# Algy/fast-slic

Measured on NVIDIA H100. Metric: megapixels/sec (10 iters, K=1600), higher is better.
Workload: dtype u8/u16 integer

## Files before the change

### fast_slic_b200/csrc/cca.cuh

```cuda
#pragma once
#include "common.cuh"

#define CCA_BLOCK 1024
#define CCA_HIST 2052

struct CcaParams {
    int H, W, N;
    int K;
    int thres;
    int nblk;
    int heap_in_smem;
    int sel_sync;
    int which;
};

__device__ __forceinline__ bool cca_skip_image(const CcaParams& cp, const struct CcaCounters* ct);

struct CcaCounters {
    int ncomp;
    int ncand;
    int nkept;
    int sel_mode;
    int keep_thres;
    int need_sim;
    int dbg_ops;
    int dbg_t;
};

__device__ __forceinline__ bool cca_skip_image(const CcaParams& cp, const CcaCounters* ct) {
    return cp.which >= 0 && (ct->need_sim != 0) != (cp.which != 0);
}

__device__ __forceinline__ int ccl_find(const int* par, int x) {
    int p = par[x];
    while (p != x) {
        x = p;
        p = par[x];
    }
    return x;
}

__device__ __forceinline__ void ccl_union(int* par, int a, int b) {
    a = ccl_find(par, a);
    b = ccl_find(par, b);
    while (a != b) {
        if (a < b) {
            int t = a;
            a = b;
            b = t;
        }
        const int old = atomicMin(&par[a], b);
        if (old == a) break;
        a = ccl_find(par, old);
        b = ccl_find(par, b);
    }
}

#define CCL_T 32
__device__ __forceinline__ int ccl_find_s(const int* par, int x) {
    int p = par[x];
    while (p != x) {
        x = p;
        p = par[x];
    }
    return x;
}
__device__ __forceinline__ void ccl_union_s(int* par, int a, int b) {
    a = ccl_find_s(par, a);
    b = ccl_find_s(par, b);
    while (a != b) {
        if (a < b) {
            int t = a;
            a = b;
            b = t;
        }
        const int old = atomicMin(&par[a], b);
        if (old == a) break;
        a = ccl_find_s(par, old);
        b = ccl_find_s(par, b);
    }
}

#define CCL_TW 4
__global__ void __launch_bounds__(32 * CCL_TW) k_ccl_tile(CcaParams cp, const uint16_t* __restrict__ labels,
                                                          int* __restrict__ par_all, uint32_t* __restrict__ area_all,
                                                          int tiles_x, int tiles_y, long ntiles_total) {
    __shared__ int s_par_all[CCL_TW][CCL_T * CCL_T];
    const int lane = threadIdx.x & 31, warp = threadIdx.x >> 5;
    const long tile = (long)blockIdx.x * CCL_TW + warp;
    if (tile >= ntiles_total) return;
    int* s_par = s_par_all[warp];
    const int per_img = tiles_x * tiles_y;
    const int b = (int)(tile / per_img);
    const int tl = (int)(tile - (long)b * per_img);
    const int tyb = tl / tiles_x, txb = tl - tyb * tiles_x;
    const int j = txb * CCL_T + lane;
    const bool colok = j < cp.W;
    const int nrows = min(CCL_T, cp.H - tyb * CCL_T);
    const uint16_t* lab = labels + (size_t)b * cp.N + (size_t)(tyb * CCL_T) * cp.W + j;
    constexpr int CCL_G = 8;
    uint32_t v[CCL_G], nv[CCL_G];
#pragma unroll
    for (int k = 0; k < CCL_G; k++) {
        v[k] = (colok && k < nrows) ? (uint32_t)lab[(size_t)k * cp.W] : (0x10000u + (uint32_t)(k * CCL_T + lane));
    }
    uint32_t up_v = 0xffffffffu, up_left = 0xffffffffu;
    int up_root = 0;
#pragma unroll 1
    for (int ty0 = 0; ty0 < CCL_T; ty0 += CCL_G) {
#pragma unroll
        for (int k = 0; k < CCL_G; k++) {
            const int ty = ty0 + CCL_G + k;
            nv[k] = (colok && ty < nrows) ? (uint32_t)lab[(size_t)ty * cp.W] : (0x10000u + (uint32_t)((ty & (CCL_T - 1)) * CCL_T + lane));
        }
#pragma unroll
        for (int k = 0; k < CCL_G; k++) {
            const int ty = ty0 + k;
            const uint32_t cur = v[k];
            const uint32_t left = __shfl_up_sync(FSLIC_FULL, cur, 1);
            const bool start = (lane == 0) || (cur != left);
            const unsigned m = __ballot_sync(FSLIC_FULL, start);
            const int sl = 31 - __clz(m & (0xffffffffu >> (31 - lane)));
            const unsigned above = (lane == 31) ? 0u : (m >> (lane + 1));
            const int end = above ? (lane + __ffs(above) - 1) : 31;
            const bool conn = (ty > 0) && (up_v == cur);
            const bool need = conn && ((lane == 0) || (left != cur) || (up_left != up_v));
            unsigned cand = 0xffffffffu;
            if (need) cand = (unsigned)ccl_find_s(s_par, up_root);
            unsigned pm = cand;
#pragma unroll
            for (int o = 1; o < 32; o <<= 1) {
                const unsigned y = __shfl_up_sync(FSLIC_FULL, pm, o);
                if (lane - o >= sl) pm = min(pm, y);
            }
            const unsigned rmin = __shfl_sync(FSLIC_FULL, pm, end);
            const unsigned own = (unsigned)(ty * CCL_T + sl);
            const int root = (int)(rmin < own ? rmin : own);
            if (need && cand != (unsigned)root) ccl_union_s(s_par, (int)cand, root);
            s_par[ty * CCL_T + lane] = root;
            __syncwarp();
            up_left = left;
            up_v = cur;
            up_root = root;
        }
#pragma unroll
        for (int k = 0; k < CCL_G; k++) v[k] = nv[k];
    }
    if (!colok) return;
    int* pout = par_all + (size_t)b * cp.N + (size_t)(tyb * CCL_T) * cp.W + j;
    uint32_t* aout = area_all + (size_t)b * cp.N + (size_t)(tyb * CCL_T) * cp.W + j;
#pragma unroll 4
    for (int ty = 0; ty < nrows; ty++) {
        const int rt = ccl_find_s(s_par, ty * CCL_T + lane);
        const int ri = tyb * CCL_T + (rt >> 5), rj = txb * CCL_T + (rt & 31);
        pout[(size_t)ty * cp.W] = ri * cp.W + rj;
        aout[(size_t)ty * cp.W] = 0;
    }
}

__global__ void __launch_bounds__(256) k_ccl_seams(CcaParams cp, const uint16_t* __restrict__ labels,
                                                   int* __restrict__ par_all) {
    const int b = blockIdx.y;
    const int W = cp.W, H = cp.H;
    const int sv = (W - 1) / CCL_T, sh = (H - 1) / CCL_T;
    const int nV = sv * H, nH = sh * W;
    const uint16_t* lab = labels + (size_t)b * cp.N;
    int* par = par_all + (size_t)b * cp.N;
    for (int t = blockIdx.x * blockDim.x + threadIdx.x; t < nV + nH; t += gridDim.x * blockDim.x) {
        if (t < nV) {
            const int i = t / sv, j = (t - i * sv + 1) * CCL_T;
            const int p = i * W + j;
            if (lab[p - 1] == lab[p]) ccl_union(par, p - 1, p);
        } else {
            const int u = t - nV;
            const int r = u / W, j = u - r * W;
            const int i = (r + 1) * CCL_T;
            const int p = i * W + j;
            const uint16_t v = lab[p], up = lab[p - W];
            if (up == v) {
                bool need = (j % CCL_T == 0) || (lab[p - 1] != v);
                if (!need) need = lab[p - W - 1] != up;
                if (need) ccl_union(par, p - W, p);
            }
        }
    }
}

__global__ void __launch_bounds__(256) k_ccl_flatten(CcaParams cp, const uint16_t* __restrict__ labels,
                                                     int* __restrict__ par_all, uint32_t* __restrict__ area_all,
                                                     int* __restrict__ blkcnt, int* __restrict__ rootbuf_all) {
    __shared__ int s_chunk[32];
    const int b = blockIdx.y;
    const int lane = threadIdx.x & 31, w = threadIdx.x >> 5;
    const uint16_t* lab = labels + (size_t)b * cp.N;
    int* par = par_all + (size_t)b * cp.N;
    int p[4], sl[4], root[4];
    unsigned m[4], rmask[4];
    bool ok[4], start[4], col0[4];
    int jcol = (blockIdx.x * CCA_BLOCK + w * 128 + lane) % cp.W;
#pragma unroll
    for (int r = 0; r < 4; r++) {
        p[r] = blockIdx.x * CCA_BLOCK + (w * 4 + r) * 32 + lane;
        ok[r] = p[r] < cp.N;
        const uint32_t v = ok[r] ? lab[p[r]] : 0x10000u;
        const uint32_t left = __shfl_up_sync(FSLIC_FULL, v, 1);
        const int j = jcol;
        col0[r] = j == 0;
        jcol += 32;
        if (jcol >= cp.W) jcol = (cp.W >= 32) ? (jcol - cp.W) : (jcol % cp.W);
        start[r] = (lane == 0) || (j == 0) || (v != left);
        m[r] = __ballot_sync(FSLIC_FULL, start[r]);
        sl[r] = 31 - __clz(m[r] & (0xffffffffu >> (31 - lane)));
    }
    {
        int q[4];
#pragma unroll
        for (int r = 0; r < 4; r++) {
            root[r] = p[r];
            q[r] = (ok[r] && start[r]) ? par[p[r]] : p[r];
        }
        for (;;) {
            bool mv[4], any = false;
#pragma unroll
            for (int r = 0; r < 4; r++) {
                mv[r] = q[r] != root[r];
                root[r] = q[r];
                any |= mv[r];
            }
            if (!any) break;
#pragma unroll
            for (int r = 0; r < 4; r++)
                if (mv[r]) q[r] = par[root[r]];
        }
    }
#pragma unroll
    for (int r = 0; r < 4; r++) {
        const int rt = __shfl_sync(FSLIC_FULL, root[r], sl[r]);
        bool isroot = false;
        if (ok[r]) {
            par[p[r]] = rt;
            if (start[r]) {
                const unsigned above = (lane == 31) ? 0u : (m[r] >> (lane + 1));
                int len = above ? (__ffs(above)) : (32 - lane);
                if (p[r] + len > cp.N) len = cp.N - p[r];
                atomicAdd(&area_all[(size_t)b * cp.N + rt], (uint32_t)len);
                isroot = (rt == p[r]);
            }
        }
        rmask[r] = __ballot_sync(FSLIC_FULL, isroot);
        if (lane == 0) s_chunk[w * 4 + r] = __popc(rmask[r]);
    }
    __syncthreads();
    const int mine = s_chunk[lane];
    int incl = mine;
#pragma unroll
    for (int o = 1; o < 32; o <<= 1) {
        const int y = __shfl_up_sync(FSLIC_FULL, incl, o);
        if (lane >= o) incl += y;
    }
    int* rootbuf = rootbuf_all + (size_t)b * cp.N + (size_t)blockIdx.x * CCA_BLOCK;
#pragma unroll
    for (int r = 0; r < 4; r++) {
        const int base = __shfl_sync(FSLIC_FULL, incl - mine, w * 4 + r);
        if ((rmask[r] >> lane) & 1u)
            rootbuf[base + __popc(rmask[r] & ((1u << lane) - 1u))] = p[r] | (col0[r] ? (int)0x80000000 : 0);
    }
    if (threadIdx.x == 31) blkcnt[(size_t)b * cp.nblk + blockIdx.x] = incl;
}

__global__ void __launch_bounds__(1024) k_scan_blocks(const int* __restrict__ cnt_all, int* __restrict__ off_all,
                                                      int stride_per_image, int n_static,
                                                      const int* __restrict__ n_dev_base, int n_dev_stride_ints,
                                                      int n_div, int* __restrict__ total_base,
                                                      int total_stride_ints,
                                                      const CcaCounters* __restrict__ skip_counters, int which) {
    __shared__ int s_warp[32];
    __shared__ int s_carry;
    const int b = blockIdx.x;
    if (skip_counters && which >= 0 && (skip_counters[b].need_sim != 0) != (which != 0)) return;
    const int tid = threadIdx.x;
    const int* cnt = cnt_all + (size_t)b * stride_per_image;
    int* off = off_all + (size_t)b * stride_per_image;
    int n = n_static;
    if (n_dev_base) n = (n_dev_base[(size_t)b * n_dev_stride_ints] + n_div - 1) / n_div;
    if (tid == 0) s_carry = 0;
    __syncthreads();
    for (int base = 0; base < n; base += 1024) {
        const int c = base + tid;
        const int v = (c < n) ? cnt[c] : 0;
        int x = v;
#pragma unroll
        for (int o = 1; o < 32; o <<= 1) {
            int y = __shfl_up_sync(FSLIC_FULL, x, o);
            if ((tid & 31) >= o) x += y;
        }
        if ((tid & 31) == 31) s_warp[tid >> 5] = x;
        __syncthreads();
        if (tid < 32) {
            int w = s_warp[tid];
#pragma unroll
            for (int o = 1; o < 32; o <<= 1) {
                int y = __shfl_up_sync(FSLIC_FULL, w, o);
                if (tid >= o) w += y;
            }
            s_warp[tid] = w;
        }
        __syncthreads();
        const int woff = (tid >> 5) ? s_warp[(tid >> 5) - 1] : 0;
        const int excl = s_carry + woff + x - v;
        if (c < n) off[c] = excl;
        __syncthreads();
        if (tid == 1023) s_carry = excl + v;
        __syncthreads();
    }
    if (tid == 0) total_base[(size_t)b * total_stride_ints] = s_carry;
}

#define CCA_NUMBER_GRID 16
__global__ void __launch_bounds__(CCA_BLOCK) k_ccl_number(CcaParams cp, const int* __restrict__ rootbuf_all,
                                                          uint32_t* __restrict__ aux_all,
                                                          const int* __restrict__ blkcnt,
                                                          const int* __restrict__ blkoff,
                                                          int* __restrict__ cleader_all,
                                                          uint32_t* __restrict__ carea_all,
                                                          CcaCounters* __restrict__ counters,
                                                          unsigned int* __restrict__ ahist_all) {
    __shared__ int s_cand;
    __shared__ unsigned int s_hot[CCA_BLOCK / 32][32];
    const int b = blockIdx.y;
    const int lane = threadIdx.x & 31, warp = threadIdx.x >> 5;
    s_hot[warp][lane] = 0;
    if (threadIdx.x == 0) s_cand = 0;
    __syncthreads();
    uint32_t* aux = aux_all + (size_t)b * cp.N;
    int ncand = 0;
    constexpr int NU = 8;
    const int wpi = gridDim.x * (CCA_BLOCK / 32);
    const int NB = (cp.nblk + wpi - 1) / wpi;
    for (int blk0 = (blockIdx.x * (CCA_BLOCK / 32) + warp) * NB; blk0 < cp.nblk; blk0 += wpi * NB) {
        for (int sub = 0; sub < NB; sub += 32) {
            const int myblk = blk0 + sub + lane;
            const bool have = (sub + lane < NB) && (myblk < cp.nblk);
            const int mycnt = have ? blkcnt[(size_t)b * cp.nblk + myblk] : 0;
            const int myoff = have ? blkoff[(size_t)b * cp.nblk + myblk] : 0;
            int incl = mycnt;
#pragma unroll
            for (int o = 1; o < 32; o <<= 1) {
                const int y = __shfl_up_sync(FSLIC_FULL, incl, o);
                if (lane >= o) incl += y;
            }
            const int total = __shfl_sync(FSLIC_FULL, incl, 31);
            const int nb_here = min(32, NB - sub);
            for (int r0 = 0; r0 < total; r0 += 32 * NU) {
                int pp[NU], cc[NU];
                uint32_t aa[NU];
#pragma unroll
                for (int u = 0; u < NU; u++) {
                    const int r = r0 + 32 * u + lane;
                    int bi = 0;
                    for (int q = 0; q < nb_here - 1; q++) bi += (r >= __shfl_sync(FSLIC_FULL, incl, q));
                    const int bincl = __shfl_sync(FSLIC_FULL, incl, bi), bcnt = __shfl_sync(FSLIC_FULL, mycnt, bi);
                    const int boff = __shfl_sync(FSLIC_FULL, myoff, bi);
                    const int t = r - (bincl - bcnt);
                    pp[u] = -1;
                    if (r < total) {
                        pp[u] = rootbuf_all[(size_t)b * cp.N + (size_t)(blk0 + sub + bi) * CCA_BLOCK + t];
                        cc[u] = boff + t;
                    }
                }
#pragma unroll
                for (int u = 0; u < NU; u++) aa[u] = pp[u] != -1 ? aux[pp[u] & 0x7fffffff] : 0u;
#pragma unroll
                for (int u = 0; u < NU; u++) {
                    uint32_t bin = 0xffffffffu;
                    if (pp[u] != -1) {
                        aux[pp[u] & 0x7fffffff] = (uint32_t)cc[u];
                        cleader_all[(size_t)b * cp.N + cc[u]] = pp[u];
                        carea_all[(size_t)b * cp.N + cc[u]] = aa[u];
                        if ((int)aa[u] >= cp.thres) bin = aa[u] < 2048u ? aa[u] : 2048u;
                    }
                    const unsigned peers = __match_any_sync(FSLIC_FULL, bin);
                    if (bin != 0xffffffffu && lane == __ffs(peers) - 1) {
                        const unsigned n = __popc(peers);
                        ncand += (int)n;
                        if (bin < 32u) s_hot[warp][bin] += n;
                        else atomicAdd(&ahist_all[(size_t)b * CCA_HIST + bin], n);
                    }
                    __syncwarp();
                }
            }
        }
    }
    ncand = __reduce_add_sync(FSLIC_FULL, ncand);
    if (lane == 0 && ncand) atomicAdd(&s_cand, ncand);
    __syncthreads();
    if (threadIdx.x == 0 && s_cand) atomicAdd(&counters[b].ncand, s_cand);
    if (threadIdx.x < 32) {
        unsigned int tot = 0;
        for (int w = 0; w < CCA_BLOCK / 32; w++) tot += s_hot[w][threadIdx.x];
        if (tot) atomicAdd(&ahist_all[(size_t)b * CCA_HIST + threadIdx.x], tot);
    }
}

__global__ void __launch_bounds__(1024) k_cca_threshold(CcaParams cp, const uint32_t* __restrict__ carea_all,
                                                        CcaCounters* __restrict__ counters,
                                                        const unsigned int* __restrict__ ahist_all) {
    __shared__ unsigned int s_hist[2048];
    __shared__ int s_warp[32];
    __shared__ unsigned int s_prefix, s_rank, s_found_bin, s_found_cnt;
    const int b = blockIdx.x;
    const int tid = threadIdx.x, lane = tid & 31, warp = tid >> 5;
    CcaCounters* ct = &counters[b];
    const int ncomp = ct->ncomp, ncand = ct->ncand;
    if (ncand <= cp.K) {
        if (tid == 0) {
            ct->keep_thres = cp.thres;
            ct->sel_mode = 0;
            ct->need_sim = 0;
        }
        return;
    }
    const uint32_t* area = carea_all + (size_t)b * cp.N;
    if (tid == 0) {
        s_prefix = 0;
        s_rank = (unsigned)cp.K;
    }
    unsigned last_E = 0;
    const unsigned int* ahist = ahist_all + (size_t)b * CCA_HIST;
    const unsigned n_big = ahist[2048];
    const bool from_hist = n_big < (unsigned)cp.K;
    int first_pass = (cp.N < (1 << 22)) ? 1 : 0;
    if (from_hist) {
        first_pass = 2;
        if (tid == 0) s_rank = (unsigned)cp.K - n_big;
        __syncthreads();
    }
    for (int pass = first_pass; pass < 3; pass++) {
        const int shift = 22 - 11 * pass;
        for (int t = tid; t < 2048; t += 1024) s_hist[t] = from_hist ? ahist[t] : 0;
        __syncthreads();
        const unsigned prefix = s_prefix;
        for (int base = 0; base < (from_hist ? 0 : ncomp); base += 4096) {
            uint32_t av[4];
#pragma unroll
            for (int u = 0; u < 4; u++) {
                const int c = base + u * 1024 + tid;
                av[u] = (c < ncomp) ? area[c] : 0xffffffffu;
            }
#pragma unroll
            for (int u = 0; u < 4; u++) {
                const uint32_t a = av[u];
                const bool valid = a != 0xffffffffu;
                const bool act = valid && ((int)a >= cp.thres) && ((pass == first_pass) || ((a >> (shift + 11)) == prefix));
                const unsigned bin = (a >> shift) & 2047u;
                const unsigned am = __ballot_sync(FSLIC_FULL, act);
                if (am) {
                    const int src = __ffs(am) - 1;
                    const unsigned b0 = __shfl_sync(FSLIC_FULL, bin, src);
                    const unsigned same = __ballot_sync(FSLIC_FULL, act && bin == b0);
                    if (lane == src) atomicAdd(&s_hist[b0], __popc(same));
                    if (act && bin != b0) atomicAdd(&s_hist[bin], 1u);
                }
            }
        }
        __syncthreads();
        const unsigned rank = s_rank;
        const int r0 = 2 * tid;
        const unsigned h0 = s_hist[2047 - r0], h1 = s_hist[2046 - r0];
        unsigned x = h0 + h1;
        const unsigned mine = x;
#pragma unroll
        for (int o = 1; o < 32; o <<= 1) {
            unsigned y = __shfl_up_sync(FSLIC_FULL, x, o);
            if (lane >= o) x += y;
        }
        if (lane == 31) s_warp[warp] = (int)x;
        __syncthreads();
        if (warp == 0) {
            unsigned w = (unsigned)s_warp[lane];
            unsigned z = w;
#pragma unroll
            for (int o = 1; o < 32; o <<= 1) {
                unsigned y = __shfl_up_sync(FSLIC_FULL, z, o);
                if (lane >= o) z += y;
            }
            s_warp[lane] = (int)(z - w);
        }
        __syncthreads();
        const unsigned before = (unsigned)s_warp[warp] + x - mine;
        if (before < rank && before + h0 >= rank) {
            s_found_bin = 2047 - r0;
            s_found_cnt = before;
        } else if (before + h0 < rank && before + h0 + h1 >= rank) {
            s_found_bin = 2046 - r0;
            s_found_cnt = before + h0;
        }
        __syncthreads();
        if (tid == 0) {
            s_prefix = (prefix << 11) | s_found_bin;
            s_rank = rank - s_found_cnt;
        }
        last_E = s_hist[s_found_bin];
        __syncthreads();
    }
    if (tid == 0) {
        const unsigned t = s_prefix;
        const unsigned need = s_rank;
        if (last_E == need) {
            ct->keep_thres = (int)t;
            ct->sel_mode = 0;
            ct->need_sim = 0;
        } else {
            ct->need_sim = 1;
        }
        ct->dbg_t = (int)t;
    }
}

#define SEL_CHUNK 8192
#define SEL_PER 8

__device__ __forceinline__ uint32_t hs_area(unsigned long long e) { return (uint32_t)(e >> 32); }

template <bool SMEM>
struct HeapMem {
    unsigned long long* g;
    uint32_t s;
    __device__ __forceinline__ void pair(int slot, uint32_t& lo0, uint32_t& hi0, uint32_t& lo1, uint32_t& hi1) const {
        if (SMEM) {
            asm volatile("ld.shared.v4.u32 {%0,%1,%2,%3}, [%4];"
                         : "=r"(lo0), "=r"(hi0), "=r"(lo1), "=r"(hi1) : "r"(s + 8u * (uint32_t)slot));
        } else {
            const uint4 v = *reinterpret_cast<const uint4*>(g + slot);
            lo0 = v.x; hi0 = v.y; lo1 = v.z; hi1 = v.w;
        }
    }
    __device__ __forceinline__ unsigned long long get(int slot) const {
        if (SMEM) {
            unsigned long long v;
            asm volatile("ld.shared.u64 %0, [%1];" : "=l"(v) : "r"(s + 8u * (uint32_t)slot));
            return v;
        }
        return g[slot];
    }
    __device__ __forceinline__ void put(int slot, uint32_t lo, uint32_t hi) const {
        if (SMEM) asm volatile("st.shared.v2.u32 [%0], {%1,%2};" :: "r"(s + 8u * (uint32_t)slot), "r"(lo), "r"(hi) : "memory");
        else g[slot] = ((unsigned long long)hi << 32) | lo;
    }
    __device__ __forceinline__ void put(int slot, unsigned long long v) const { put(slot, (uint32_t)v, (uint32_t)(v >> 32)); }
};

template <bool SMEM>
__device__ __forceinline__ void hs_adjust_heap(const HeapMem<SMEM>& h, int hole, int len, unsigned long long value) {
    const uint32_t va = hs_area(value);
    for (;;) {
        const int l = 2 * hole + 1;
        if (l >= len) break;
        uint32_t lo0, hi0, lo1, hi1;
        h.pair(l + 1, lo0, hi0, lo1, hi1);
        const bool take_left = (l + 1 >= len) || (hi1 > hi0);
        const uint32_t clo = take_left ? lo0 : lo1, chi = take_left ? hi0 : hi1;
        if (chi > va) break;
        h.put(hole + 1, clo, chi);
        hole = take_left ? l : l + 1;
    }
    h.put(hole + 1, value);
}

#define SEL_CHILDREN "ld.volatile.shared.v4.u32 {a0, a1, b0, b1}, [c];\n\t"
#define SEL_HALF_STEP(BAR)                                                                                  \
    "setp.gt.u32 tl, b1, a1;\n\t"                         \
    "min.u32 chi, a1, b1;\n\t"                                                                            \
    "selp.b32 clo, a0, b0, tl;\n\t"                                                                       \
    "setp.le.and.u32 mv, chi, vhi, act;\n\t"                  \
    "min.u32 ohi, chi, vhi;\n\t"                                                                          \
    "selp.b32 olo, clo, vlo, mv;\n\t"                                                                     \
    "@act st.volatile.shared.v2.u32 [hole], {olo, ohi};\n\t"              \
    BAR                                                                                                   \
    "add.u32 c8, c, 8;\n\t"                                                                               \
    "selp.b32 nh, c, c8, tl;\n\t"                                                                         \
    "selp.b32 hole, nh, rooth, mv;\n\t"       \
    "add.u32 t0, hole, hole;\n\t"                                                                         \
    "sub.u32 c, t0, base;\n\t"                          \
    "mov.pred act, mv;\n\t"

#define SEL_LOOP_ASM(BAR)                                                                                                   \
    "{\n\t"                                                                                                                 \
    ".reg .pred act, mv, tl, p, some, first, nact, take, kill, inq;\n\t"                                                    \
    ".reg .b32 base, c, hole, vlo, vhi, a0, a1, b0, b1, chi, clo, ohi, olo, c8, nh, t0, t1, t2, root, hit, elo, ehi;\n\t"    \
    ".reg .b32 lt, le, wpos, idx, qaddr, rooth, drain;\n\t"                                                                 \
    "mov.u32 base, %2;\n\t"                                                                                                 \
    "mov.u32 lt, %%lanemask_lt;\n\t"                                                                                        \
    "mov.u32 le, %%lanemask_le;\n\t"                                                                                        \
    "add.u32 rooth, base, 8;\n\t"                                             \
    "mov.u32 hole, rooth;\n\t"                                                                                              \
    "add.u32 c, base, 16;\n\t"                                                                                              \
    "mov.u32 vlo, 0;\n\t"                                                                                                   \
    "mov.u32 vhi, 0;\n\t"                                                                                                   \
    "setp.ne.u32 act, 0, 0;\n\t"                                                                                            \
    "mov.u32 wpos, %5;\n\t"                                                                                                 \
    SEL_CHILDREN                                                                                                            \
    "SEL_LOAD:\n\t"                                    \
    "add.u32 idx, wpos, %6;\n\t"                                                                                            \
    "setp.lt.s32 inq, idx, %4;\n\t"                                                                                         \
    "mov.u32 elo, 0;\n\t"                                                                                                   \
    "mov.u32 ehi, 0;\n\t"                                     \
    "shl.b32 qaddr, idx, 3;\n\t"                                                                                            \
    "add.u32 qaddr, qaddr, %3;\n\t"                                                                                         \
    "@inq ld.shared.v2.u32 {elo, ehi}, [qaddr];\n\t"                                                                        \
    "SEL_TRIP:\n\t"                                                                                                         \
    "add.u32 %1, %1, 1;\n\t"                                                                                                \
    SEL_HALF_STEP(BAR)                                      \
    "ld.volatile.shared.u32 root, [base+12];\n\t"                         \
    SEL_CHILDREN                                                                                                            \
    SEL_HALF_STEP(BAR)                                                                                                      \
    "setp.gt.u32 p, ehi, root;\n\t"                                                    \
    "vote.sync.ballot.b32 hit, p, 0xffffffff;\n\t"                                                                          \
    "vote.sync.any.pred some, p, 0xffffffff;\n\t"                                                                           \
    SEL_CHILDREN                            \
                                             \
    "@!some bra.uni SEL_NEXT;\n\t"                                                                                          \
    "and.b32 t1, hit, lt;\n\t"                                                                                              \
    "setp.eq.and.u32 first, t1, 0, p;\n\t"                                                                                  \
    "not.pred nact, act;\n\t"                                                                                               \
    "and.pred take, first, nact;\n\t"                                                                                       \
    "and.b32 t2, hit, le;\n\t"                                                                                              \
    "setp.eq.or.u32 kill, t2, 0, take;\n\t"                       \
    "@take mov.u32 vlo, elo;\n\t"                                                                                           \
    "@take mov.u32 vhi, ehi;\n\t"                                                                                           \
    "@take add.u32 %0, %0, 1;\n\t"                                                                                          \
    "@kill mov.u32 ehi, 0;\n\t"                                                                                             \
    "or.pred act, act, take;\n\t"                                                                                           \
    "bra.uni SEL_TRIP;\n\t"                                                                                                 \
    "SEL_NEXT:\n\t"                                 \
    "add.u32 wpos, wpos, 32;\n\t"                                                                                           \
    "setp.lt.s32 inq, wpos, %4;\n\t"                                                                                        \
    "@inq bra.uni SEL_LOAD;\n\t"                                                                                            \
    "mov.u32 drain, %7;\n\t"                                           \
    "SEL_DRAIN:\n\t"                                                                                                        \
    SEL_HALF_STEP(BAR)                                                                                                      \
    SEL_CHILDREN                                                                                                            \
    "sub.u32 drain, drain, 1;\n\t"                                                                                          \
    "setp.gt.s32 inq, drain, 0;\n\t"                                                                                        \
    "@inq bra.uni SEL_DRAIN;\n\t"                                                                                           \
    "}\n\t"

template <bool WARPSYNC>
__device__ __forceinline__ int sel_replay_smem(uint32_t heap_saddr, uint32_t queue_saddr, int qn, int consumed, int depth, int lane,
                                               long long& trips_out) {
    uint32_t cnt = 0, trips = 0;
    if (consumed < qn) {
        if (WARPSYNC)
            asm volatile(SEL_LOOP_ASM("bar.warp.sync 0xffffffff;\n\t")
                         : "+r"(cnt), "+r"(trips)
                         : "r"(heap_saddr), "r"(queue_saddr), "r"(qn), "r"(consumed), "r"(lane), "r"(depth)
                         : "memory");
        else
            asm volatile(SEL_LOOP_ASM("")
                         : "+r"(cnt), "+r"(trips)
                         : "r"(heap_saddr), "r"(queue_saddr), "r"(qn), "r"(consumed), "r"(lane), "r"(depth)
                         : "memory");
        __syncwarp();
    }
    trips_out = trips;
    return (int)__reduce_add_sync(FSLIC_FULL, cnt);
}

template <bool SMEM, bool WARPSYNC = true>
__device__ __forceinline__ void heap_select_body(const uint32_t* __restrict__ area, int ncomp, int K, int thres,
                                                  const HeapMem<SMEM> heap, uint32_t* __restrict__ mark_out ,
                                                  uint8_t* __restrict__ kept_bytes ,
                                                  unsigned long long* s_queue ,
                                                  int* dbg_ops = nullptr, long long* prof = nullptr ) {
    __shared__ int s_warp[32];
    __shared__ int s_qn, s_filled;
    __shared__ uint32_t s_min;
    const int tid = threadIdx.x, lane = tid & 31, warp = tid >> 5, nt = blockDim.x;
    if (tid == 0) {
        s_filled = 0;
        s_min = 0;
    }
    if (SMEM)
        for (int u = K + 1 + tid; u < 2 * K + 4; u += nt) heap.put(u, 0u, 0xffffffffu);
    __syncthreads();
    long long pt_filter = 0, pt_build = 0, pt_replay = 0, pn_iter = 0, pn_queue = 0, pn_chunks = 0, pt0 = clock64(), pt_mark = pt0;
    uint32_t cur[SEL_PER], nxt[SEL_PER];
#pragma unroll
    for (int u = 0; u < SEL_PER; u++) {
        const int c = tid * SEL_PER + u;
        cur[u] = (c < ncomp) ? area[c] : 0u;
    }
    for (int base = 0; base < ncomp; base += SEL_CHUNK) {
#pragma unroll
        for (int u = 0; u < SEL_PER; u++) {
            const int c = base + SEL_CHUNK + tid * SEL_PER + u;
            nxt[u] = (c < ncomp) ? area[c] : 0u;
        }
        const int filled = s_filled;
        const bool filling = filled < K;
        const uint32_t curmin = s_min;
        int cnt = 0;
#pragma unroll
        for (int u = 0; u < SEL_PER; u++) {
            const int c = base + tid * SEL_PER + u;
            cnt += (c < ncomp) && ((int)cur[u] >= thres) && (filling || cur[u] > curmin);
        }
        int x = cnt;
#pragma unroll
        for (int o = 1; o < 32; o <<= 1) {
            int y = __shfl_up_sync(FSLIC_FULL, x, o);
            if (lane >= o) x += y;
        }
        if (lane == 31) s_warp[warp] = x;
        __syncthreads();
        if (warp == 0) {
            int w = (lane < (nt >> 5)) ? s_warp[lane] : 0;
            int z = w;
#pragma unroll
            for (int o = 1; o < 32; o <<= 1) {
                int y = __shfl_up_sync(FSLIC_FULL, z, o);
                if (lane >= o) z += y;
            }
            s_warp[lane] = z - w;
            if (lane == 31) s_qn = z;
        }
        __syncthreads();
        int pos = s_warp[warp] + x - cnt;
#pragma unroll
        for (int u = 0; u < SEL_PER; u++) {
            const int c = base + tid * SEL_PER + u;
            if ((c < ncomp) && ((int)cur[u] >= thres) && (filling || cur[u] > curmin))
                s_queue[pos++] = ((unsigned long long)cur[u] << 32) | (uint32_t)c;
        }
        __syncthreads();
        const int qn = s_qn;
        if (prof && tid == 0) {
            const long long now = clock64();
            pt_filter += now - pt_mark;
            pt_mark = now;
            pn_queue += qn;
            pn_chunks++;
        }
        int consumed = 0;
        if (filling) {
            consumed = min(qn, K - filled);
            for (int u = tid; u < consumed; u += nt) heap.put(filled + u + 1, s_queue[u]);
            __syncthreads();
        }
        const int f = filled + consumed;
        if (filling && f == K && K >= 2) {
            const int last_parent = (K - 2) / 2;
            int lvl = 31 - __clz(last_parent + 1);
            for (; lvl >= 0; lvl--) {
                const int lo = (1 << lvl) - 1, hi = min((2 << lvl) - 2, last_parent);
                for (int node = lo + tid; node <= hi; node += nt) hs_adjust_heap(heap, node, K, heap.get(node + 1));
                __syncthreads();
            }
        }
        if (prof && tid == 0) {
            const long long now = clock64();
            pt_build += now - pt_mark;
            pt_mark = now;
        }
        if (f == K && warp == 0) {
            int nops = 0;
            if (SMEM) {
                long long trips = 0;
                nops = sel_replay_smem<WARPSYNC>(heap.s, (uint32_t)__cvta_generic_to_shared(s_queue), qn, consumed, 32 - __clz(K), lane, trips);
                pn_iter += trips;
            } else {
            bool act = false;
            int hole = 0;
            uint32_t vlo = 0, vhi = 0;
            int qpos = consumed, next_lane = 0;
            const int depth = 32 - __clz(K);
            int idle = depth;
            const uint32_t q_saddr = (uint32_t)__cvta_generic_to_shared(s_queue);
            auto level_step = [&]() {
                const int l = 2 * hole + 1;
                const bool inb = act && (l < K);
                uint32_t lo0, hi0, lo1, hi1;
                heap.pair(inb ? l + 1 : 2, lo0, hi0, lo1, hi1);
                const bool take_left = (l + 1 >= K) || (hi1 > hi0);
                const uint32_t clo = take_left ? lo0 : lo1, chi = take_left ? hi0 : hi1;
                const bool move = inb && !(chi > vhi);
                if (act) heap.put(hole + 1, move ? clo : vlo, move ? chi : vhi);
                hole = move ? (take_left ? l : l + 1) : hole;
                act = move;
                __syncwarp();
            };
            while (qpos < qn || idle < depth) {
                level_step();
                uint32_t elo = 0, ehi = 0, root_area = 0xffffffffu;
                const bool have = qpos < qn;
                if (have) {
                    asm volatile("ld.shared.v2.u32 {%0,%1}, [%2];" : "=r"(elo), "=r"(ehi) : "r"(q_saddr + 8u * (uint32_t)qpos));
                    root_area = hs_area(heap.get(1));
                }
                level_step();
                idle += 2;
                if (have) {
                    qpos++;
                    if (ehi > root_area) {
                        if (lane == next_lane) {
                            act = true;
                            hole = 0;
                            vlo = elo;
                            vhi = ehi;
                        }
                        next_lane = (next_lane + 1) & 31;
                        nops++;
                        idle = 0;
                    }
                }
            }
            }
            if (lane == 0) {
                s_min = hs_area(heap.get(1));
                if (dbg_ops) *dbg_ops += nops;
                if (prof) {
                    const long long now = clock64();
                    pt_replay += now - pt_mark;
                    pt_mark = now;
                }
            }
        }
        if (tid == 0) s_filled = f;
        __syncthreads();
#pragma unroll
        for (int u = 0; u < SEL_PER; u++) cur[u] = nxt[u];
    }
    if (prof && tid == 0) {
        prof[0] = clock64() - pt0;
        prof[1] = pt_filter;
        prof[2] = pt_build;
        prof[3] = pt_replay;
        prof[4] = pn_iter;
        prof[5] = pn_queue;
        prof[6] = pn_chunks;
        prof[7] = ncomp;
    }
    const int filled = s_filled;
    for (int u = tid; u < filled; u += nt) {
        const uint32_t c = (uint32_t)(heap.get(u + 1) & 0xffffffffu);
        if (mark_out) mark_out[c] |= 0x80000000u;
        if (kept_bytes) kept_bytes[c] = 1;
    }
}

__global__ void __launch_bounds__(1024) k_cca_select(CcaParams cp, uint32_t* __restrict__ carea_all,
                                                     CcaCounters* __restrict__ counters,
                                                     unsigned long long* __restrict__ heap_global, long long* __restrict__ prof_all) {
    extern __shared__ __align__(16) unsigned char sel_smem[];
    unsigned long long* s_queue = reinterpret_cast<unsigned long long*>(sel_smem);
    const int b = blockIdx.x;
    CcaCounters* ct = &counters[b];
    if (!ct->need_sim) return;
    uint32_t* area = carea_all + (size_t)b * cp.N;
    long long* prof = prof_all ? prof_all + 8 * b : nullptr;
    if (cp.heap_in_smem) {
        HeapMem<true> hm;
        hm.g = nullptr;
        hm.s = (uint32_t)__cvta_generic_to_shared(sel_smem + SEL_CHUNK * 8);
        if (cp.sel_sync) heap_select_body<true, true>(area, ct->ncomp, cp.K, cp.thres, hm, area, nullptr, s_queue, &ct->dbg_ops, prof);
        else heap_select_body<true, false>(area, ct->ncomp, cp.K, cp.thres, hm, area, nullptr, s_queue, &ct->dbg_ops, prof);
    } else {
        HeapMem<false> hm;
        hm.g = heap_global + (size_t)b * ((cp.K + 3) & ~1);
        hm.s = 0;
        heap_select_body<false>(area, ct->ncomp, cp.K, cp.thres, hm, area, nullptr, s_queue, &ct->dbg_ops, prof);
    }
    if (threadIdx.x == 0) ct->sel_mode = 1;
}

__global__ void __launch_bounds__(1024) k_debug_heap_select(const uint32_t* __restrict__ area, int n, int middle,
                                                            uint8_t* __restrict__ kept,
                                                            unsigned long long* __restrict__ heap_global, int use_smem) {
    extern __shared__ __align__(16) unsigned char sel_smem[];
    unsigned long long* s_queue = reinterpret_cast<unsigned long long*>(sel_smem);
    if (use_smem) {
        HeapMem<true> hm;
        hm.g = nullptr;
        hm.s = (uint32_t)__cvta_generic_to_shared(sel_smem + SEL_CHUNK * 8);
        heap_select_body<true>(area, n, middle, 0, hm, nullptr, kept, s_queue);
    } else {
        HeapMem<false> hm;
        hm.g = heap_global;
        hm.s = 0;
        heap_select_body<false>(area, n, middle, 0, hm, nullptr, kept, s_queue);
    }
}

__device__ __forceinline__ bool cca_is_kept(uint32_t a, int sel_mode, int keep_thres) {
    return sel_mode ? (a >> 31) : ((int)a >= keep_thres);
}

#define CCA_KEPT_GRID 16
#define CCA_KEPT_U 4
__global__ void __launch_bounds__(CCA_BLOCK) k_kept_count(CcaParams cp, const uint32_t* __restrict__ carea_all,
                                                          const CcaCounters* __restrict__ counters,
                                                          int* __restrict__ blkcnt) {
    __shared__ int s_cnt[CCA_KEPT_U];
    const int b = blockIdx.y;
    if (cca_skip_image(cp, &counters[b])) return;
    const int ncomp = counters[b].ncomp;
    const int sel_mode = counters[b].sel_mode, keep_thres = counters[b].keep_thres;
    const uint32_t* carea = carea_all + (size_t)b * cp.N;
    for (int blk0 = blockIdx.x * CCA_KEPT_U; blk0 * CCA_BLOCK < ncomp; blk0 += gridDim.x * CCA_KEPT_U) {
        if (threadIdx.x < CCA_KEPT_U) s_cnt[threadIdx.x] = 0;
        uint32_t a[CCA_KEPT_U];
#pragma unroll
        for (int u = 0; u < CCA_KEPT_U; u++) {
            const int c = (blk0 + u) * CCA_BLOCK + threadIdx.x;
            a[u] = (c < ncomp) ? carea[c] : 0u;
        }
        __syncthreads();
#pragma unroll
        for (int u = 0; u < CCA_KEPT_U; u++) {
            const int c = (blk0 + u) * CCA_BLOCK + threadIdx.x;
            const bool kept = (c < ncomp) && cca_is_kept(a[u], sel_mode, keep_thres);
            const unsigned m = __ballot_sync(FSLIC_FULL, kept);
            if ((threadIdx.x & 31) == 0 && m) atomicAdd(&s_cnt[u], __popc(m));
        }
        __syncthreads();
        if (threadIdx.x < CCA_KEPT_U && (blk0 + threadIdx.x) * CCA_BLOCK < ncomp)
            blkcnt[(size_t)b * cp.nblk + blk0 + threadIdx.x] = s_cnt[threadIdx.x];
        __syncthreads();
    }
}

__global__ void __launch_bounds__(CCA_BLOCK) k_kept_label(CcaParams cp, const uint32_t* __restrict__ carea_all,
                                                          const CcaCounters* __restrict__ counters,
                                                          const int* __restrict__ blkoff,
                                                          uint16_t* __restrict__ cnew_all) {
    __shared__ int s_warp[CCA_KEPT_U][32];
    const int b = blockIdx.y;
    if (cca_skip_image(cp, &counters[b])) return;
    const int ncomp = counters[b].ncomp;
    const int sel_mode = counters[b].sel_mode, keep_thres = counters[b].keep_thres;
    const int tid = threadIdx.x, lane = tid & 31, warp = tid >> 5;
    const uint32_t* carea = carea_all + (size_t)b * cp.N;
    for (int blk0 = blockIdx.x * CCA_KEPT_U; blk0 * CCA_BLOCK < ncomp; blk0 += gridDim.x * CCA_KEPT_U) {
        uint32_t a[CCA_KEPT_U];
        int off[CCA_KEPT_U];
#pragma unroll
        for (int u = 0; u < CCA_KEPT_U; u++) {
            const int c = (blk0 + u) * CCA_BLOCK + tid;
            a[u] = (c < ncomp) ? carea[c] : 0u;
            off[u] = ((blk0 + u) * CCA_BLOCK < ncomp) ? blkoff[(size_t)b * cp.nblk + blk0 + u] : 0;
        }
        unsigned m[CCA_KEPT_U];
        bool kept[CCA_KEPT_U];
        __syncthreads();
#pragma unroll
        for (int u = 0; u < CCA_KEPT_U; u++) {
            const int c = (blk0 + u) * CCA_BLOCK + tid;
            kept[u] = (c < ncomp) && cca_is_kept(a[u], sel_mode, keep_thres);
            m[u] = __ballot_sync(FSLIC_FULL, kept[u]);
            if (lane == 0) s_warp[u][warp] = __popc(m[u]);
        }
        __syncthreads();
        if (warp < CCA_KEPT_U) {
            const int w = s_warp[warp][lane];
            int x = w;
#pragma unroll
            for (int o = 1; o < 32; o <<= 1) {
                const int y = __shfl_up_sync(FSLIC_FULL, x, o);
                if (lane >= o) x += y;
            }
            s_warp[warp][lane] = x - w;
        }
        __syncthreads();
#pragma unroll
        for (int u = 0; u < CCA_KEPT_U; u++) {
            const int c = (blk0 + u) * CCA_BLOCK + tid;
            if (c < ncomp) {
                uint16_t v = 0xFFFF;
                if (kept[u]) v = (uint16_t)(off[u] + s_warp[u][warp] + __popc(m[u] & ((1u << lane) - 1)));
                cnew_all[(size_t)b * cp.N + c] = v;
            }
        }
    }
}

__global__ void __launch_bounds__(256) k_cca_absorb(CcaParams cp, const int* __restrict__ par_all,
                                                    const uint32_t* __restrict__ aux_all,
                                                    const int* __restrict__ cleader_all,
                                                    const uint16_t* __restrict__ cnew_all,
                                                    const CcaCounters* __restrict__ counters,
                                                    uint16_t* __restrict__ final_all) {
    const int b = blockIdx.y;
    if (cca_skip_image(cp, &counters[b])) return;
    const int ncomp = counters[b].ncomp;
    const int* par = par_all + (size_t)b * cp.N;
    const uint32_t* aux = aux_all + (size_t)b * cp.N;
    const int* cleader = cleader_all + (size_t)b * cp.N;
    const uint16_t* cnew = cnew_all + (size_t)b * cp.N;
    for (int c0 = blockIdx.x * blockDim.x + threadIdx.x; c0 < ncomp; c0 += gridDim.x * blockDim.x) {
    int c = c0;
    uint16_t lab = cnew[c];
    while (lab == 0xFFFF) {
        if (c == 0) {
            lab = 0;
            break;
        }
        const int lf = cleader[c], l = lf & 0x7fffffff;
        const int q = (lf >= 0) ? (l - 1) : (l - cp.W);
        c = (int)aux[par[q]];
        lab = cnew[c];
    }
    final_all[(size_t)b * cp.N + (cleader[c0] & 0x7fffffff)] = lab;
    }
}

__global__ void __launch_bounds__(256) k_cca_output(CcaParams cp, const int* __restrict__ par_all,
                                                    const uint16_t* __restrict__ final_all,
                                                    uint16_t* __restrict__ out_all,
                                                    const CcaCounters* __restrict__ counters) {
    const int b = blockIdx.y;
    if (cca_skip_image(cp, &counters[b])) return;
    const int* par = par_all + (size_t)b * cp.N;
    const uint16_t* fin = final_all + (size_t)b * cp.N;
    uint16_t* out = out_all + (size_t)b * cp.N;
    if ((cp.N & 7) == 0 && (reinterpret_cast<uintptr_t>(out_all) & 15) == 0 && (reinterpret_cast<uintptr_t>(par_all) & 15) == 0) {
        for (int t = blockIdx.x * blockDim.x + threadIdx.x; t < cp.N / 8; t += gridDim.x * blockDim.x) {
            const int4 r0 = reinterpret_cast<const int4*>(par)[2 * t], r1 = reinterpret_cast<const int4*>(par)[2 * t + 1];
            const uint32_t a0 = fin[r0.x];
            uint32_t a1 = a0, a2, a3, a4, a5, a6, a7;
            if (r0.y != r0.x) a1 = fin[r0.y];
            a2 = a1; if (r0.z != r0.y) a2 = fin[r0.z];
            a3 = a2; if (r0.w != r0.z) a3 = fin[r0.w];
            a4 = a3; if (r1.x != r0.w) a4 = fin[r1.x];
            a5 = a4; if (r1.y != r1.x) a5 = fin[r1.y];
            a6 = a5; if (r1.z != r1.y) a6 = fin[r1.z];
            a7 = a6; if (r1.w != r1.z) a7 = fin[r1.w];
            reinterpret_cast<uint4*>(out)[t] = make_uint4(a0 | (a1 << 16), a2 | (a3 << 16), a4 | (a5 << 16), a6 | (a7 << 16));
        }
        return;
    }
    for (int p = blockIdx.x * blockDim.x + threadIdx.x; p < cp.N; p += gridDim.x * blockDim.x) out[p] = fin[par[p]];
}
```

Before: 15640.

## Accumulate component areas per tile in shared memory before global flatten

Moves area counting into the tile CCL kernel: each row run adds its length into the high 16 bits of the shared parent entry, and tile-local roots write their partial areas. The flatten kernel then does one global atomicAdd per tile-local root that is not a global root, instead of one per run, which cuts global atomics. It also replaces launch_bounds with a 48-register cap. The risk is extra per-row work in the tile kernel and register spills.

```diff
diff --git a/fast_slic_b200/csrc/cca.cuh b/fast_slic_b200/csrc/cca.cuh
--- a/fast_slic_b200/csrc/cca.cuh
+++ b/fast_slic_b200/csrc/cca.cuh
@@ -82,7 +82,7 @@
 }
 
 #define CCL_TW 4
-__global__ void __launch_bounds__(32 * CCL_TW) k_ccl_tile(CcaParams cp, const uint16_t* __restrict__ labels,
+__global__ void __maxnreg__(48) k_ccl_tile(CcaParams cp, const uint16_t* __restrict__ labels,
                                                           int* __restrict__ par_all, uint32_t* __restrict__ area_all,
                                                           int tiles_x, int tiles_y, long ntiles_total) {
     __shared__ int s_par_all[CCL_TW][CCL_T * CCL_T];
@@ -146,15 +146,38 @@
 #pragma unroll
         for (int k = 0; k < CCL_G; k++) v[k] = nv[k];
     }
-    if (!colok) return;
     int* pout = par_all + (size_t)b * cp.N + (size_t)(tyb * CCL_T) * cp.W + j;
     uint32_t* aout = area_all + (size_t)b * cp.N + (size_t)(tyb * CCL_T) * cp.W + j;
+    const int ncols = min(CCL_T, cp.W - txb * CCL_T);
+#pragma unroll 1
+    for (int ty = 0; ty < nrows; ty++) {
+        int rt = ty * CCL_T + lane;
+        if (colok) {
+            int q = s_par[rt] & 0xffff;
+            while (q != rt) {
+                rt = q;
+                q = s_par[rt] & 0xffff;
+            }
+        }
+        const int left = __shfl_up_sync(FSLIC_FULL, rt, 1);
+        const bool start = (lane == 0) || !colok || (left != rt);
+        const unsigned m = __ballot_sync(FSLIC_FULL, start);
+        if (colok) {
+            const int ri = tyb * CCL_T + (rt >> 5), rj = txb * CCL_T + (rt & 31);
+            pout[(size_t)ty * cp.W] = ri * cp.W + rj;
+            if (start) {
+                const unsigned above = (lane == 31) ? 0u : (m >> (lane + 1));
+                const int len = above ? __ffs(above) : (ncols - lane);
+                atomicAdd(&s_par[rt], len << 16);
+            }
+        }
+        __syncwarp();
+    }
+    if (!colok) return;
 #pragma unroll 4
     for (int ty = 0; ty < nrows; ty++) {
-        const int rt = ccl_find_s(s_par, ty * CCL_T + lane);
-        const int ri = tyb * CCL_T + (rt >> 5), rj = txb * CCL_T + (rt & 31);
-        pout[(size_t)ty * cp.W] = ri * cp.W + rj;
-        aout[(size_t)ty * cp.W] = 0;
+        const int e = s_par[ty * CCL_T + lane];
+        aout[(size_t)ty * cp.W] = ((e & 0xffff) == ty * CCL_T + lane) ? (uint32_t)e >> 16 : 0u;
     }
 }
 
@@ -195,7 +218,7 @@
     const uint16_t* lab = labels + (size_t)b * cp.N;
     int* par = par_all + (size_t)b * cp.N;
     int p[4], sl[4], root[4];
-    unsigned m[4], rmask[4];
+    unsigned m[4], rmask[4], tarea[4];
     bool ok[4], start[4], col0[4];
     int jcol = (blockIdx.x * CCA_BLOCK + w * 128 + lane) % cp.W;
 #pragma unroll
@@ -209,6 +232,7 @@
         jcol += 32;
         if (jcol >= cp.W) jcol = (cp.W >= 32) ? (jcol - cp.W) : (jcol % cp.W);
         start[r] = (lane == 0) || (j == 0) || (v != left);
+        tarea[r] = (ok[r] && (start[r] || (j & (CCL_T - 1)) == 0)) ? area_all[(size_t)b * cp.N + p[r]] : 0u;
         m[r] = __ballot_sync(FSLIC_FULL, start[r]);
         sl[r] = 31 - __clz(m[r] & (0xffffffffu >> (31 - lane)));
     }
@@ -239,13 +263,8 @@
         bool isroot = false;
         if (ok[r]) {
             par[p[r]] = rt;
-            if (start[r]) {
-                const unsigned above = (lane == 31) ? 0u : (m[r] >> (lane + 1));
-                int len = above ? (__ffs(above)) : (32 - lane);
-                if (p[r] + len > cp.N) len = cp.N - p[r];
-                atomicAdd(&area_all[(size_t)b * cp.N + rt], (uint32_t)len);
-                isroot = (rt == p[r]);
-            }
+            if (tarea[r] != 0u && rt != p[r]) atomicAdd(&area_all[(size_t)b * cp.N + rt], tarea[r]);
+            isroot = start[r] && (rt == p[r]);
         }
         rmask[r] = __ballot_sync(FSLIC_FULL, isroot);
         if (lane == 0) s_chunk[w * 4 + r] = __popc(rmask[r]);
```

Measured after the change: 16020 (median of 6 runs). About the same (+2.4%).
